# burlachenkok/flpytorch

Measured on AMD Instinct MI355X. Metric: gradient-codec encode+reduce GB/s (device-resident), [N,D] fp32; % HBM peak, higher is better.
Workload: dtype f32; 1 GPU; C3 topk:1% N=1024/GPU D=10000000; codec=topk:1%, clients_per_gpu=1024, clients_total=1024, D=10000000, K=100000, rows_alloc=contiguous, parallelism=client-shard dp1

## Files before the change

flpytorch_amd/csrc/select.hip:

```cpp
#include <stdlib.h>

#include <atomic>
#include <map>
#include <mutex>
#include <vector>

#include "chunks.hpp"
#include "randk_tree.hpp"

namespace flc {

constexpr uint32_t ALL = 0xFFFFFFFFu;
constexpr uint32_t F_OVERFLOW = 1u, F_SHORT = 2u, F_TIES = 4u, F_EXACT = 8u;
constexpr uint32_t F_RESIDENT = 16u;
constexpr uint32_t F_REPAIR = 32u;
constexpr int SMAX = 16384;
constexpr int HBINS = 2048;
constexpr uint32_t TIECAP = HBINS;
constexpr int CS_SH = 64;
constexpr int64_t CS_FEW = 16;
constexpr int CS_ST = 8;
constexpr int CS_LCAP = 2048;
constexpr int RS_U = 16;
#ifndef FLC_RS_NG
#define FLC_RS_NG 4
#endif
constexpr int RS_NG = FLC_RS_NG;
constexpr int RS_NG_MAX = 16;
static_assert(RS_NG >= 1 && RS_NG <= RS_NG_MAX, "FLC_RS_NG: 1..16 groups");
constexpr int RS_GLOB = 0, RS_GEN = 32, RS_GAVE = 64, RS_CCNT = 96, RS_CDONE = 112, RS_GRP = 128;
constexpr int RS_XGRP = RS_GRP + 32 * RS_NG_MAX;
constexpr int RS_ABV = RS_XGRP + 32 * RS_NG_MAX;
constexpr int RS_CAP = 2048;
constexpr int RS_SS = 8192;
#ifndef FLC_RS_SR
#define FLC_RS_SR 1
#endif
constexpr int RS_SR = FLC_RS_SR;
#ifndef FLC_RS_STPOL
#define FLC_RS_STPOL 2
#endif
#ifndef FLC_RS_GACQ
#define FLC_RS_GACQ 1
#endif
#ifndef FLC_RS_POLLAB
#define FLC_RS_POLLAB 1
#endif
#ifndef FLC_RS_DONE
#define FLC_RS_DONE 1
#endif
#ifndef FLC_RS_RANKFIRST
#define FLC_RS_RANKFIRST 0
#endif
#ifndef FLC_RS_PROBE_NOCOUNT
#define FLC_RS_PROBE_NOCOUNT 0
#endif
#ifndef FLC_RS_G0REL
#define FLC_RS_G0REL 1
#endif
#ifndef FLC_RS_FENCE
#define FLC_RS_FENCE 0
#endif
#ifndef FLC_RS_SPEC
#define FLC_RS_SPEC 1
#endif
constexpr int RS_HREP = RS_ABV + 32 * RS_NG_MAX;
constexpr int RS_HSPEC = RS_HREP + 3 * RS_NG * HBINS;
constexpr int RS_CLIST = RS_HSPEC + 3 * RS_NG * HBINS;
constexpr int RS_TCNT = RS_CLIST + 2 * RS_CAP;
constexpr int RS_GMAX = 1024;
constexpr int RS_CS = 4;
constexpr int RS_CNUM = RS_TCNT + 2 * RS_GMAX;
constexpr int RS_CREG = RS_CNUM + RS_GMAX;
#ifdef FLC_RS_PRINT
constexpr int RS_PROBE = RS_CREG + 2 * RS_CS * RS_GMAX;
constexpr int RS_CTL = RS_PROBE + 4096;
#else
constexpr int RS_CTL = RS_CREG + 2 * RS_CS * RS_GMAX;
#endif
#ifndef FLC_RS_SPECST
#define FLC_RS_SPECST 0
#endif
#ifndef FLC_CS_LIST
#define FLC_CS_LIST 1
#endif
#ifndef FLC_CS_TWO_MAXD
#define FLC_CS_TWO_MAXD (int64_t(64) << 20)
#endif

struct SelWs {
    uint2* tab;
    uint32_t* ent_idx;
    float* ent_val;
    uint32_t* rowcnt;
    uint32_t* flags;
    uint32_t* thr;
    uint32_t* prefix;
    uint32_t* krem;
    uint32_t* tieprefix;
    uint32_t* tiecut;
    uint32_t* hist;
    uint32_t* worklist;
    uint32_t* nwork;
    uint32_t* cursor;
    uint32_t* cstate;
    uint64_t* clist;
    uint32_t* carrive;
    uint32_t* shcnt;
    uint32_t* zm;
    float* part;
    int64_t cap;
    uint32_t tie_hi;
};

__device__ __host__ inline uint32_t tie_pref(uint32_t ix, uint32_t hi) { return hi ? ix : ~ix; }
__device__ __host__ inline uint32_t tie_all(uint32_t hi) { return hi ? 0u : 0xFFFFFFFFu; }


__device__ inline void lds_bar() {
    asm volatile("s_waitcnt lgkmcnt(0)" ::: "memory");
    __builtin_amdgcn_s_barrier();
    asm volatile("" ::: "memory");
}
template <bool RAW>
__device__ inline void blk_bar() {
    if (RAW) lds_bar();
    else __syncthreads();
}
template <bool RAW = false>
__device__ inline void hist_find_at(const uint32_t* h, uint32_t k, uint32_t& bin, uint32_t& above,
                                    uint32_t* scratch , int t, bool own) {
    uint32_t local[8];
    uint32_t s = 0;
#pragma unroll
    for (int q = 0; q < 8; ++q) { local[q] = own ? h[HBINS - 1 - (t * 8 + q)] : 0u; s += local[q]; }
    if (t == 0) { scratch[256] = 0; scratch[257] = 0; }
    const int lane = t & 63, w = t >> 6;
    uint32_t inc = s;
#pragma unroll
    for (int off = 1; off < 64; off <<= 1) {
        const uint32_t v = __shfl_up(inc, off, 64);
        inc += lane >= off ? v : 0u;
    }
    if (own && lane == 63) scratch[w] = inc;
    blk_bar<RAW>();
    uint32_t before = 0;
    if (own)
        for (int q = 0; q < w; ++q) before += scratch[q];
    uint32_t incl = own ? before + inc : 0u, excl = incl - s;
    if (own && excl < k && incl >= k) {
        uint32_t run = excl;
#pragma unroll
        for (int q = 0; q < 8; ++q) {
            if (run + local[q] >= k) {
                scratch[256] = (uint32_t)(HBINS - 1 - (t * 8 + q));
                scratch[257] = run;
                break;
            }
            run += local[q];
        }
    }
    blk_bar<RAW>();
    bin = scratch[256];
    above = scratch[257];
    blk_bar<RAW>();
}
template <int NB>
__device__ inline void hist_find_n(const uint32_t* h, uint32_t k, uint32_t& bin, uint32_t& above, bool& found,
                                   uint32_t* scratch ) {
    constexpr int PER = NB / 256;
    static_assert(NB % 256 == 0, "256 threads scan NB / 256 bins each");
    const int t = (int)threadIdx.x;
    const bool own = t < 256;
    uint32_t local[PER];
    uint32_t s = 0;
#pragma unroll
    for (int q = 0; q < PER; ++q) { local[q] = own ? h[NB - 1 - (t * PER + q)] : 0u; s += local[q]; }
    if (t == 0) { scratch[256] = 0; scratch[257] = 0; scratch[258] = 0; }
    const int lane = t & 63, w = t >> 6;
    uint32_t inc = s;
#pragma unroll
    for (int off = 1; off < 64; off <<= 1) {
        const uint32_t v = __shfl_up(inc, off, 64);
        inc += lane >= off ? v : 0u;
    }
    if (own && lane == 63) scratch[w] = inc;
    __syncthreads();
    uint32_t before = 0;
    if (own)
        for (int q = 0; q < w; ++q) before += scratch[q];
    const uint32_t incl = own ? before + inc : 0u, excl = incl - s;
    if (own && excl < k && incl >= k) {
        uint32_t run = excl;
#pragma unroll
        for (int q = 0; q < PER; ++q) {
            if (run + local[q] >= k) {
                scratch[256] = (uint32_t)(NB - 1 - (t * PER + q));
                scratch[257] = run;
                scratch[258] = 1;
                break;
            }
            run += local[q];
        }
    }
    __syncthreads();
    bin = scratch[256];
    above = scratch[257];
    found = scratch[258] != 0u;
    __syncthreads();
}
template <bool RAW = false>
__device__ inline void hist_find(const uint32_t* h, uint32_t k, uint32_t& bin, uint32_t& above,
                                 uint32_t* scratch ) {
    hist_find_at<RAW>(h, k, bin, above, scratch, (int)threadIdx.x, threadIdx.x < 256);
}
__device__ inline void hist_find2(const uint32_t* ha, uint32_t ka, uint32_t& bina, uint32_t& abovea, uint32_t* sa,
                                  const uint32_t* hb, uint32_t kb, uint32_t& binb, uint32_t& aboveb, uint32_t* sb) {
    const bool second = threadIdx.x >= 256;
    uint32_t bin, above;
    hist_find_at(second ? hb : ha, second ? kb : ka, bin, above, second ? sb : sa, (int)(threadIdx.x & 255u),
                 threadIdx.x < 512);
    bina = sa[256]; abovea = sa[257];
    binb = sb[256]; aboveb = sb[257];
    __syncthreads();
}

__device__ inline uint32_t pass_shift(int p) { return p == 0 ? 20u : (p == 1 ? 9u : 0u); }
__device__ inline uint32_t pass_bits(int p) { return p == 2 ? 9u : 11u; }
__device__ inline bool key_in_prefix(uint32_t key, int p, uint32_t prefix) {
    if (p == 0) return true;
    uint32_t sh = pass_shift(p) + pass_bits(p);
    return (key >> sh) == prefix;
}
__device__ inline uint32_t key_bin(uint32_t key, int p) {
    return (key >> pass_shift(p)) & ((1u << pass_bits(p)) - 1u);
}

template <int NT, bool DUAL>
__global__ __launch_bounds__(NT) void k_topk_sample(RowSrc rows, int64_t n, int64_t d, int64_t K, SelWs ws, int few,
                                                    int64_t r_off) {
    __shared__ uint32_t keys[SMAX];
    __shared__ uint32_t h[HBINS], h2[DUAL ? HBINS : 1];
    __shared__ uint32_t scratch[260], scratch2[DUAL ? 260 : 1];
    const int64_t row = r_off + blockIdx.x;
    if (row >= n) return;
    const float* r = rows.row(row);
    int S;
    if (d <= SMAX) {
        S = (int)d;
        for (int i = threadIdx.x; i < S; i += NT) keys[i] = mag_key(r[i]);
    } else {
        const int P = SMAX / 256;
        S = SMAX;
        constexpr int GR = NT / 256, PU = 32 / GR;
        const int e = threadIdx.x & 255, g0 = threadIdx.x >> 8;
        for (int p0 = 0; p0 < P; p0 += 32) {
            float x[PU];
#pragma unroll
            for (int u = 0; u < PU; ++u) x[u] = r[((int64_t)(p0 + u * GR + g0) * (d - 256)) / (P - 1) + e];
#pragma unroll
            for (int u = 0; u < PU; ++u) keys[(p0 + u * GR + g0) * 256 + e] = mag_key(x[u]);
        }
    }
    const int NP = S == d ? 3 : 2;
    uint32_t rank;
    if (S == d) {
        rank = (uint32_t)K;
    } else {
        double ks = (double)K * (double)S / (double)d;
        double rr = ks + 4.0 * sqrt(ks) + 8.0;
        rank = (uint32_t)min((double)S, ceil(rr));
    }
    static_assert(!DUAL || NT >= 512, "hist_find2 takes 512 threads");
    auto rank_key = [&](uint32_t r) {
        uint32_t prefix = 0, krem = r;
        for (int p = 0; p < NP; ++p) {
            for (int i = threadIdx.x; i < HBINS; i += NT) h[i] = 0;
            __syncthreads();
            for (int i = threadIdx.x; i < S; i += NT) {
                uint32_t k = keys[i];
                if (key_in_prefix(k, p, prefix)) atomicAdd(&h[key_bin(k, p)], 1u);
            }
            __syncthreads();
            uint32_t bin, above;
            hist_find(h, krem, bin, above, scratch);
            prefix = (prefix << pass_bits(p)) | bin;
            krem -= above;
            __syncthreads();
        }
        return NP == 3 ? prefix : prefix << 9;
    };
    auto rank_keys = [&](uint32_t ra, uint32_t rb, uint32_t& ka, uint32_t& kb) {
        if constexpr (!DUAL) {
            ka = rank_key(ra);
            kb = rb == ra ? ka : rank_key(rb);
            return;
        }
        uint32_t pa = 0, pb = 0, ma = ra, mb = rb;
        for (int p = 0; p < NP; ++p) {
            const bool same = pa == pb;
            for (int i = threadIdx.x; i < HBINS; i += NT) { h[i] = 0; h2[i] = 0; }
            __syncthreads();
            for (int i = threadIdx.x; i < S; i += NT) {
                const uint32_t k = keys[i];
                if (key_in_prefix(k, p, pa)) atomicAdd(&h[key_bin(k, p)], 1u);
                if (!same && key_in_prefix(k, p, pb)) atomicAdd(&h2[key_bin(k, p)], 1u);
            }
            __syncthreads();
            uint32_t ba, aa, bb, ab;
            hist_find2(h, ma, ba, aa, scratch, same ? h : h2, mb, bb, ab, scratch2);
            pa = (pa << pass_bits(p)) | ba;
            ma -= aa;
            pb = (pb << pass_bits(p)) | bb;
            mb -= ab;
        }
        ka = NP == 3 ? pa : pa << 9;
        kb = NP == 3 ? pb : pb << 9;
    };
    uint32_t tkey, kest;
    rank_keys(rank, S == d ? rank : (uint32_t)max(1.0, min((double)S, (double)K * (double)S / (double)d)), tkey, kest);
    if (threadIdx.x == 0) {
        ws.thr[row] = (rank >= (uint32_t)S && S != d) ? 0u : tkey;
        ws.prefix[row] = kest;
        ws.flags[row] = 0;
        ws.rowcnt[(row) * RCS] = 0;
        if (few) { ws.cstate[row * CS_ST + 3] = 0; ws.cstate[row * CS_ST + 5] = 0; ws.carrive[row * RCS] = 0; }
    }
    if (few && threadIdx.x < CS_SH) ws.shcnt[(row * CS_SH + threadIdx.x) * RCS] = 0;
    if (few)
        for (int i = threadIdx.x; i < HBINS; i += NT) ws.hist[row * HBINS + i] = 0;
}

#ifndef FLC_CS_NT
#define FLC_CS_NT 1
#endif
__device__ inline float4 cs_ld(const float4* p) {
#if FLC_CS_NT
    typedef float v4f __attribute__((ext_vector_type(4)));
    const v4f v = __builtin_nontemporal_load(reinterpret_cast<const v4f*>(p));
    return make_float4(v.x, v.y, v.z, v.w);
#else
    return *p;
#endif
}
template <int NT>
__device__ void cand_select_row(int64_t row, int64_t K, SelWs ws, uint32_t* h, uint32_t* scratch) {
    {
        if (ws.flags[row]) return;
        const uint32_t cnt = ws.rowcnt[(row) * RCS];
        if (cnt < (uint32_t)K) {
            if (threadIdx.x == 0) ws.flags[row] |= F_SHORT;
            return;
        }
        const uint32_t T = ws.thr[row];
        const uint32_t span = ws.prefix[row] - T;
        int s = 0;
        while (s < 21 && (((uint64_t)span * 4u) >> s) >= (uint64_t)HBINS) ++s;
        const float* vals = ws.ent_val + row * ws.cap;
        const float4* v4 = reinterpret_cast<const float4*>(vals);
        const uint32_t n4 = cnt >> 2;
        uint32_t prefix = 0, krem = (uint32_t)K, last = 0;
        bool first = true, fail = false;
        int sh = s;
        while (true) {
            const int s1 = first ? sh : max(0, sh - 11);
            const uint32_t mask = first ? 0xFFFFFFFFu : ((1u << (sh - s1)) - 1u);
            for (int i = threadIdx.x; i < HBINS; i += NT) h[i] = 0;
            __syncthreads();
            auto add = [&](float x) {
                const uint32_t dk = mag_key(x) - T;
                if (first) atomicAdd(&h[min(dk >> s1, (uint32_t)(HBINS - 1))], 1u);
                else if ((dk >> sh) == prefix) atomicAdd(&h[(dk >> s1) & mask], 1u);
            };
            uint32_t i = threadIdx.x;
            for (; i + 7 * NT < n4; i += 8 * NT) {
                float4 q[8];
#pragma unroll
                for (int u = 0; u < 8; ++u) q[u] = cs_ld(v4 + i + u * NT);
#pragma unroll
                for (int u = 0; u < 8; ++u) { add(q[u].x); add(q[u].y); add(q[u].z); add(q[u].w); }
            }
            for (; i < n4; i += NT) {
                const float4 q = v4[i];
                add(q.x); add(q.y); add(q.z); add(q.w);
            }
            for (uint32_t i = n4 * 4 + threadIdx.x; i < cnt; i += NT) add(vals[i]);
            __syncthreads();
            uint32_t bin, above;
            hist_find(h, krem, bin, above, scratch);
            last = h[bin];
            if (first && bin == HBINS - 1) { fail = true; break; }
            prefix = first ? bin : ((prefix << (sh - s1)) | bin);
            krem -= above;
            sh = s1;
            first = false;
            __syncthreads();
            if (sh == 0) break;
        }
        __syncthreads();
        const uint32_t thr = T + prefix;
        bool ties = !fail && last > krem;
        if (ties && last > TIECAP) { fail = true; ties = false; }
        if (ties) {
            uint32_t* tix = h;
            if (threadIdx.x == 0) scratch[0] = 0;
            __syncthreads();
            const uint32_t* idxs = ws.ent_idx + row * ws.cap;
            for (uint32_t i = threadIdx.x; i < n4; i += NT) {
                const float4 q = v4[i];
                const float qv[4] = {q.x, q.y, q.z, q.w};
#pragma unroll
                for (int u = 0; u < 4; ++u)
                    if (mag_key(qv[u]) == thr) tix[atomicAdd(&scratch[0], 1u)] = idxs[i * 4 + u];
            }
            for (uint32_t i = n4 * 4 + threadIdx.x; i < cnt; i += NT) {
                if (mag_key(vals[i]) == thr) tix[atomicAdd(&scratch[0], 1u)] = idxs[i];
            }
            __syncthreads();
            const uint32_t m = scratch[0];
            for (uint32_t a = threadIdx.x; a < m; a += NT) {
                const uint32_t ia = tix[a];
                uint32_t rank = 0;
                for (uint32_t b = 0; b < m; ++b) rank += tie_pref(tix[b], ws.tie_hi) > tie_pref(ia, ws.tie_hi) ? 1u : 0u;
                if (rank == krem - 1) ws.tiecut[row] = ia;
            }
        }
        if (threadIdx.x == 0) {
            if (fail) {
                ws.flags[row] |= F_SHORT;
            } else {
                ws.thr[row] = thr;
                ws.krem[row] = krem;
                if (ties) ws.flags[row] |= F_TIES;
            }
        }
        __syncthreads();
    }
}

template <int NT>
__global__ __launch_bounds__(NT) void k_cand_select(int64_t r0, int64_t rn, int64_t K, SelWs ws) {
    __shared__ uint32_t h[HBINS];
    __shared__ uint32_t scratch[260];
    for (int64_t row = r0 + blockIdx.x; row < r0 + rn; row += gridDim.x) {
        cand_select_row<NT>(row, K, ws, h, scratch);
        __syncthreads();
    }
}

constexpr int CS_NT = 256;
__global__ __launch_bounds__(CS_NT) void k_cs_pass(int64_t K, SelWs ws, int final_pass) {
    __shared__ uint32_t h[HBINS];
    __shared__ uint32_t scratch[260];
    __shared__ uint32_t last_wg;
    __shared__ uint64_t lst[FLC_CS_LIST ? CS_LCAP : 1];
    const int64_t row = blockIdx.y;
    const uint32_t B = gridDim.x, b = blockIdx.x;
    uint32_t* cs = ws.cstate + row * CS_ST;
    const uint32_t stage = cs[3];
    if (stage >= 2u) return;
    const uint32_t* shc = ws.shcnt + row * CS_SH * RCS;
    uint32_t cnt = 0;
    for (int k = 0; k < CS_SH; ++k) cnt += shc[k * RCS];
    const uint32_t mycnt = shc[b * RCS];
    const bool first = stage == 0u;
    if (first && (ws.flags[row] != 0u || cnt < (uint32_t)K)) {
        if (b == 0 && threadIdx.x == 0) {
            if (ws.flags[row] == 0u) ws.flags[row] = F_SHORT;
            cs[3] = 2u;
        }
        return;
    }
    const uint32_t T = ws.thr[row];
    uint32_t sh, prefix, krem;
    if (first) {
        const uint32_t span = ws.prefix[row] - T;
        uint32_t s0 = 0;
        while (s0 < 21 && (((uint64_t)span * 4u) >> s0) >= (uint64_t)HBINS) ++s0;
        sh = s0; prefix = 0; krem = (uint32_t)K;
    } else {
        sh = cs[0]; prefix = cs[1]; krem = cs[2];
    }
    const uint32_t s1 = first ? sh : (sh > 11u ? sh - 11u : 0u);
    const uint32_t mask = first ? 0xFFFFFFFFu : ((1u << (sh - s1)) - 1u);
    const int64_t segcap = (ws.cap / CS_SH) & ~int64_t(3);
    if (FLC_CS_LIST && !first && cs[4] <= (uint32_t)CS_LCAP) {
        if (threadIdx.x == 0) scratch[0] = 0;
        __syncthreads();
        const float* sv = ws.ent_val + row * ws.cap + b * segcap;
        const uint32_t* si = ws.ent_idx + row * ws.cap + b * segcap;
        for (uint32_t e = threadIdx.x; e < mycnt; e += CS_NT) {
            const uint32_t key = mag_key(sv[e]);
            if (((key - T) >> sh) == prefix) {
                const uint32_t slot = atomicAdd(&scratch[0], 1u);
                if (slot < (uint32_t)CS_LCAP) lst[slot] = ((uint64_t)key << 32) | (uint64_t)tie_pref(si[e], ws.tie_hi);
            }
        }
        __syncthreads();
        const uint32_t nl = min(scratch[0], (uint32_t)CS_LCAP);
        if (threadIdx.x == 0) scratch[1] = nl ? atomicAdd(&cs[5], nl) : 0u;
        __syncthreads();
        uint64_t* gl = ws.clist + row * CS_LCAP;
        const uint32_t gb = scratch[1];
        for (uint32_t i = threadIdx.x; i < nl; i += CS_NT)
            if (gb + i < (uint32_t)CS_LCAP) gl[gb + i] = lst[i];
        asm volatile("s_waitcnt vmcnt(0)" ::: "memory");
        __syncthreads();
        if (threadIdx.x == 0) {
            __builtin_amdgcn_fence(__ATOMIC_RELEASE, "agent");
            last_wg = atomicAdd(&ws.carrive[row * RCS], 1u) == B - 1u ? 1u : 0u;
        }
        __syncthreads();
        if (!last_wg) return;
        __builtin_amdgcn_fence(__ATOMIC_ACQUIRE, "agent");
        const uint32_t m = __hip_atomic_load(&cs[5], __ATOMIC_RELAXED, __HIP_MEMORY_SCOPE_AGENT);
        const bool ok = m == cs[4] && m >= krem && krem >= 1u;
        const uint32_t mm = min(m, (uint32_t)CS_LCAP);
        for (uint32_t i = threadIdx.x; i < mm; i += CS_NT)
            lst[i] = __hip_atomic_load(&gl[i], __ATOMIC_RELAXED, __HIP_MEMORY_SCOPE_AGENT);
        if (threadIdx.x == 0) { scratch[0] = 0; scratch[1] = 0; scratch[2] = 0; scratch[3] = 0; }
        __syncthreads();
        if (ok)
            for (uint32_t i = threadIdx.x; i < mm; i += CS_NT) {
                const uint64_t me = lst[i];
                uint32_t rank = 0;
                for (uint32_t j = 0; j < mm; ++j) rank += lst[j] > me ? 1u : 0u;
                if (rank == krem - 1u) { scratch[0] = (uint32_t)(me >> 32); scratch[1] = tie_pref((uint32_t)me, ws.tie_hi); }
            }
        __syncthreads();
        const uint32_t kth = scratch[0];
        if (ok)
            for (uint32_t i = threadIdx.x; i < mm; i += CS_NT) {
                const uint32_t key = (uint32_t)(lst[i] >> 32);
                if (key > kth) atomicAdd(&scratch[2], 1u);
                else if (key == kth) atomicAdd(&scratch[3], 1u);
            }
        __syncthreads();
        if (threadIdx.x == 0) {
            atomicExch(&ws.carrive[row * RCS], 0u);
            if (!ok) {
                ws.flags[row] |= F_SHORT;
            } else {
                const uint32_t gt = scratch[2], eq = scratch[3];
                ws.thr[row] = kth;
                ws.krem[row] = krem - gt;
                if (gt + eq > krem) { ws.tiecut[row] = scratch[1]; ws.flags[row] |= F_TIES; }
            }
            cs[3] = 2u;
        }
        return;
    }
    for (int i = threadIdx.x; i < HBINS; i += CS_NT) h[i] = 0;
    __syncthreads();
    auto add = [&](float x) {
        const uint32_t dk = mag_key(x) - T;
        if (first) atomicAdd(&h[min(dk >> s1, (uint32_t)(HBINS - 1))], 1u);
        else if ((dk >> sh) == prefix) atomicAdd(&h[(dk >> s1) & mask], 1u);
    };
    const float* vals = ws.ent_val + row * ws.cap + b * segcap;
    const float4* v4 = reinterpret_cast<const float4*>(vals);
    const uint32_t n4 = mycnt >> 2, q1 = n4;
    uint32_t i = threadIdx.x;
    for (; i + 3 * CS_NT < q1; i += 4 * CS_NT) {
        float4 q[4];
#pragma unroll
        for (int u = 0; u < 4; ++u) q[u] = cs_ld(v4 + i + u * CS_NT);
#pragma unroll
        for (int u = 0; u < 4; ++u) { add(q[u].x); add(q[u].y); add(q[u].z); add(q[u].w); }
    }
    for (; i < q1; i += CS_NT) {
        const float4 q = cs_ld(v4 + i);
        add(q.x); add(q.y); add(q.z); add(q.w);
    }
    for (uint32_t t = n4 * 4 + threadIdx.x; t < mycnt; t += CS_NT) add(vals[t]);
    __syncthreads();
    uint32_t* gh = ws.hist + row * HBINS;
    for (int t = threadIdx.x; t < HBINS; t += CS_NT)
        if (h[t]) atomicAdd(gh + t, h[t]);
    asm volatile("s_waitcnt vmcnt(0)" ::: "memory");
    __syncthreads();
    if (threadIdx.x == 0) {
        __builtin_amdgcn_fence(__ATOMIC_RELEASE, "agent");
        asm volatile("s_waitcnt vmcnt(0)" ::: "memory");
        last_wg = atomicAdd(&ws.carrive[row * RCS], 1u) == B - 1u ? 1u : 0u;
    }
    __syncthreads();
// ... 265 lines not shown
#pragma unroll
    for (int L = 0; L < RING - 1; ++L) {
        ring[L] = load_q(rs, lane, L);
        __builtin_amdgcn_sched_barrier(0);
    }
    const int64_t segcap = shards > 1 ? (ws.cap / shards) & ~int64_t(3) : ws.cap;
    bool pv = false;
    int64_t prow = 0, pc0 = 0, pseg = 0;
    uint64_t pcc = 0;
    uint32_t ptot = 0, pres = 0;
    int par = 0;
    auto finish = [&](int pb) {
        uint32_t base = 0;
        bool fits = ptot <= GCAP;
        if (fits && ptot) {
            base = __shfl(pres, 0, WAVE);
            fits = (int64_t)base + ptot <= segcap;
            base += (uint32_t)(pseg * segcap);
        }
        if (lane < FGS && pc0 + lane < C) {
            uint32_t off = 0, cc = 0;
#pragma unroll
            for (int u = 0; u < FGS; ++u) {
                const uint32_t cu = (uint32_t)(pcc >> (16 * u)) & 0xFFFFu;
                off += u < lane ? cu : 0u;
                cc = u == lane ? cu : cc;
            }
            ws.tab[(pc0 + lane) * n + prow] = make_uint2(base + off, fits ? cc : 0u);
        }
        if (!fits && lane == 0) atomicOr(&ws.flags[prow], F_OVERFLOW);
#if FLC_TK_COPY4
        tk_copy_out(st[pb][wv], st[pb][wv] + SROW, ws, n, prow, base, ptot, fits, lane, (int64_t)blockIdx.x * 4 + wv);
#else
        if (fits && FLC_TK_PROBE != 2) {
            const uint32_t* si = st[pb][wv];
            const float* sv = reinterpret_cast<const float*>(st[pb][wv] + SROW);
            uint32_t* oi = ws.ent_idx + prow * ws.cap + base;
            float* ov = ws.ent_val + prow * ws.cap + base;
#pragma unroll
            for (int k = 0; k < GCAP / 64; ++k) {
                const uint32_t e = (uint32_t)(k * 64 + lane);
                if (e < ptot) { oi[e] = si[e]; ov[e] = sv[e]; }
            }
        }
#endif
    };
    while (it < items) {
        const uint32_t T = max(sload(ws.thr + row), 1u);
        const int64_t nit = it + stride;
        const uint32_t sla = __builtin_amdgcn_readfirstlane((uint32_t)(size_t)(__attribute__((address_space(3))) uint32_t*)st[par][wv]);
        uint32_t cnt = 0;
        uint64_t ccp = 0;
        const int64_t cg0 = c;
        int64_t nrow = row, nc = c;
#pragma unroll
        for (int sub = 0; sub < FGS; ++sub, ++c) {
            const int64_t j0 = c * CHUNK;
            __amdgpu_buffer_rsrc_t rsn;
            if (sub + 1 < FGS) {
                rsn = chunk_rsrc(rows.row_s(row), j0 + CHUNK, d);
            } else if (nit < items) {
                item_at(nit, nrow, nc);
                rsn = chunk_rsrc(rows.row_s(nrow), nc * CHUNK, d);
            } else {
                rsn = __builtin_amdgcn_make_buffer_rsrc(const_cast<float*>(rows.row_s(row)), (short)0, 0, 0x00020000);
            }
            const uint32_t cnt0 = cnt;
            __amdgpu_buffer_rsrc_t ro;
            if constexpr (LONE != 0) ro = chunk_rsrc(zout, j0, d);
            uint32_t lb = (uint32_t)j0 + (uint32_t)lane * 4u;
            asm volatile("" : "+v"(lb));
#pragma unroll
            for (int L = 0; L < 16; ++L) {
                const int P = L + RING - 1;
                ring[P % RING] = P < 16 ? load_q(rs, lane, P) : load_q(rsn, lane, P - 16);
                const float4 x = ring[L % RING];
                if constexpr (LONE != 0) {
                    typedef unsigned int u4v __attribute__((ext_vector_type(4)));
                    const u4v z = {0u, 0u, 0u, 0u};
                    __builtin_amdgcn_raw_buffer_store_b128(z, ro, lane * 16, L * 1024, 0);
                }
                const uint32_t jl = lb + (uint32_t)(L * 256);
                const float vq[4] = {x.x, x.y, x.z, x.w};
#pragma unroll
                for (int q = 0; q < 4; ++q) {
                    if (FLC_TK_PROBE == 3) { cnt += __float_as_uint(vq[q]) == 0x7F800001u ? 1u : 0u; continue; }
                    const bool f = mag_key(vq[q]) >= T;
                    const uint64_t m = __ballot(f);
                    if (FLC_TK_PROBE != 1 && f) {
                        const uint32_t pre = __builtin_amdgcn_mbcnt_hi((uint32_t)(m >> 32), __builtin_amdgcn_mbcnt_lo((uint32_t)m, 0u));
                        uint32_t sb = sla + min(cnt, (uint32_t)GCAP) * 4u;
                        asm volatile("" : "+s"(sb));
                        asm volatile("ds_write2st64_b32 %0, %1, %2 offset1:%3" ::"v"(sb + pre * 4u),
                                     "v"(jl + q), "v"(__float_as_uint(vq[q])), "i"(SROW * 4 / 256) : "memory");
                    }
                    cnt += (uint32_t)__popcll(m);
                }
            }
            ccp |= (uint64_t)min(cnt - cnt0, 0xFFFFu) << (16 * (c - cg0));
            rs = rsn;
        }
        if (pv) finish(par ^ 1);
        uint32_t res = 0;
        const int64_t shard = shards > 1 ? (cg0 / FGS) % shards : 0;
        if (cnt && cnt <= GCAP && lane == 0)
            res = atomicAdd(shards > 1 ? &ws.shcnt[(row * shards + shard) * RCS] : &ws.rowcnt[(row) * RCS], cnt);
        pv = true; prow = row; pc0 = cg0; pcc = ccp; ptot = cnt; pres = res; pseg = shard;
        __builtin_amdgcn_fence(__ATOMIC_SEQ_CST, "wavefront");
        par ^= 1;
        it = nit;
        row = nrow;
        c = nc;
    }
    __builtin_amdgcn_fence(__ATOMIC_SEQ_CST, "wavefront");
    finish(par ^ 1);
}

#ifndef FLC_TK_WG
#define FLC_TK_WG 1
#endif
#ifndef FLC_TK_WG_NL
#define FLC_TK_WG_NL 4
#endif
#ifndef FLC_TK_WG_RING
#define FLC_TK_WG_RING FLC_TK_RING
#endif
#ifndef FLC_TK_WG_STPOL
#define FLC_TK_WG_STPOL 17
#endif
#ifndef FLC_TK_WG_WPE
#define FLC_TK_WG_WPE 4
#endif
__device__ inline uint32_t lds_addr(const void* p) {
    return (uint32_t)(size_t)(const __attribute__((address_space(3))) void*)p;
}
__device__ inline uint32_t lds_peek(uint32_t addr) {
    uint32_t v;
    asm volatile("ds_read_b32 %0, %1\n\ts_waitcnt lgkmcnt(0)" : "=&v"(v) : "v"(addr) : "memory");
    return __builtin_amdgcn_readfirstlane(v);
}
template <int RING, int NL>
__global__ __launch_bounds__((NL + 1) * 64) __attribute__((amdgpu_waves_per_eu(FLC_TK_WG_WPE))) void k_topk_filter_fast_wg(RowSrc rows, int64_t n, int64_t r0, int64_t rn, int64_t rb, int64_t d,
                                                                        SelWs ws) {
    static_assert(16 % RING == 0, "ring must divide the 16 loads of a chunk");
    constexpr int FGS = 4;
    constexpr int SROW = GCAP + 64;
    __shared__ __attribute__((aligned(16))) uint32_t st[2][NL][2 * SROW];
    __shared__ __attribute__((aligned(16))) uint32_t hs[2][NL][4];
    __shared__ uint32_t fr[2];
    const int lane = threadIdx.x & 63;
    const int wv = __builtin_amdgcn_readfirstlane(threadIdx.x >> 6);
    if (threadIdx.x < 2 * NL * 4) (&hs[0][0][0])[threadIdx.x] = 0;
    if (threadIdx.x < 2) fr[threadIdx.x] = 0;
    __syncthreads();
    const int64_t C = nchunks(d);
    const int64_t G = (C + FGS * NL - 1) / (FGS * NL);
    const int64_t items = rn * G;
    const int64_t stride = gridDim.x;
    int64_t it = blockIdx.x;
    if (it >= items) return;
    auto item_at = [&](int64_t t, int64_t& r, int64_t& cc) {
        const int64_t blk = t / (rb * G), rem = t - blk * rb * G;
        const int64_t bn = min(rb, rn - blk * rb);
        const int64_t g = rem / bn;
        r = r0 + blk * rb + (rem - g * bn);
        cc = g * (FGS * NL);
    };
    if (wv == NL) {
        for (uint32_t k = 0; it < items; it += stride, ++k) {
            const int b = k & 1;
            int64_t row, c0;
            item_at(it, row, c0);
            const uint32_t fa = lds_addr(&hs[b][min(lane, NL - 1)][3]);
            for (;;) {
                uint32_t f;
                asm volatile("ds_read_b32 %0, %1\n\ts_waitcnt lgkmcnt(0)" : "=&v"(f) : "v"(fa) : "memory");
                if (__ballot(f != k + 1) == 0) break;
                __builtin_amdgcn_s_sleep(4);
            }
            uint32_t pre[NL], tot[NL], sum = 0;
            uint64_t cc[NL];
            bool allfit = true;
#pragma unroll
            for (int w = 0; w < NL; ++w) {
                const uint4 h = *reinterpret_cast<const uint4*>(hs[b][w]);
                cc[w] = (uint64_t)h.x | ((uint64_t)h.y << 32);
                tot[w] = h.z;
                pre[w] = sum;
                sum += tot[w] <= GCAP ? tot[w] : 0u;
                allfit = allfit && tot[w] <= GCAP;
            }
            uint32_t base = 0;
            bool fits = true;
            if (sum) {
                uint32_t res = 0;
                if (lane == 0) res = atomicAdd(&ws.rowcnt[row * RCS], sum);
                base = __shfl(res, 0, WAVE);
                fits = (int64_t)base + sum <= ws.cap;
            }
            if (lane < FGS * NL && c0 + lane < C) {
                uint32_t off = 0, cu = 0;
                bool gf = false;
#pragma unroll
                for (int w = 0; w < NL; ++w)
                    if ((lane >> 2) == w) {
                        off = pre[w];
                        gf = tot[w] <= GCAP;
#pragma unroll
                        for (int u = 0; u < FGS; ++u) {
                            const uint32_t x = (uint32_t)(cc[w] >> (16 * u)) & 0xFFFFu;
                            off += u < (lane & 3) ? x : 0u;
                            cu = u == (lane & 3) ? x : cu;
                        }
                    }
                ws.tab[(c0 + lane) * n + row] = make_uint2(base + off, fits && gf ? cu : 0u);
            }
            if (!(fits && allfit) && lane == 0) atomicOr(&ws.flags[row], F_OVERFLOW);
#pragma unroll
            for (int w = 0; w < NL; ++w)
                tk_copy_out<FLC_TK_WG_STPOL>(st[b][w], st[b][w] + SROW, ws, n, row, base + pre[w], tot[w], fits && tot[w] <= GCAP, lane,
                            (int64_t)blockIdx.x * NL + w);
            asm volatile("s_waitcnt lgkmcnt(0)\n\tds_write_b32 %0, %1" ::"v"(lds_addr(&fr[b])), "v"(k + 1) : "memory");
        }
        return;
    }
    float4 ring[RING];
    int64_t row, c;
    item_at(it, row, c);
    c += wv * FGS;
    auto rs = chunk_rsrc(rows.row_s(row), c * CHUNK, d);
#pragma unroll
    for (int L = 0; L < RING - 1; ++L) {
        ring[L] = load_q(rs, lane, L);
        __builtin_amdgcn_sched_barrier(0);
    }
    for (uint32_t k = 0; it < items; ++k) {
        const int b = k & 1;
        if (k >= 2) {
            const uint32_t fa = lds_addr(&fr[b]);
            while (lds_peek(fa) != k - 1) __builtin_amdgcn_s_sleep(2);
        }
        const uint32_t T = max(sload(ws.thr + row), 1u);
        const int64_t nit = it + stride;
        const uint32_t sla = __builtin_amdgcn_readfirstlane(lds_addr(st[b][wv]));
        uint32_t cnt = 0;
        uint64_t ccp = 0;
        const int64_t cg0 = c;
        int64_t nrow = row, nc = c;
#pragma unroll
        for (int sub = 0; sub < FGS; ++sub, ++c) {
            const int64_t j0 = c * CHUNK;
            __amdgpu_buffer_rsrc_t rsn;
            if (sub + 1 < FGS) {
                rsn = chunk_rsrc(rows.row_s(row), j0 + CHUNK, d);
            } else if (nit < items) {
                item_at(nit, nrow, nc);
                nc += wv * FGS;
                rsn = chunk_rsrc(rows.row_s(nrow), nc * CHUNK, d);
            } else {
                rsn = __builtin_amdgcn_make_buffer_rsrc(const_cast<float*>(rows.row_s(row)), (short)0, 0, 0x00020000);
            }
            const uint32_t cnt0 = cnt;
            uint32_t lb = (uint32_t)j0 + (uint32_t)lane * 4u;
            asm volatile("" : "+v"(lb));
#pragma unroll
            for (int L = 0; L < 16; ++L) {
                const int P = L + RING - 1;
                ring[P % RING] = P < 16 ? load_q(rs, lane, P) : load_q(rsn, lane, P - 16);
                const float4 x = ring[L % RING];
                const uint32_t jl = lb + (uint32_t)(L * 256);
                const float vq[4] = {x.x, x.y, x.z, x.w};
#pragma unroll
                for (int q = 0; q < 4; ++q) {
                    const bool f = mag_key(vq[q]) >= T;
                    const uint64_t m = __ballot(f);
                    if (f) {
                        const uint32_t pre = __builtin_amdgcn_mbcnt_hi((uint32_t)(m >> 32), __builtin_amdgcn_mbcnt_lo((uint32_t)m, 0u));
                        uint32_t sb = sla + min(cnt, (uint32_t)GCAP) * 4u;
                        asm volatile("" : "+s"(sb));
                        asm volatile("ds_write2st64_b32 %0, %1, %2 offset1:%3" ::"v"(sb + pre * 4u),
                                     "v"(jl + q), "v"(__float_as_uint(vq[q])), "i"(SROW * 4 / 256) : "memory");
                    }
                    cnt += (uint32_t)__popcll(m);
                }
            }
            ccp |= (uint64_t)min(cnt - cnt0, 0xFFFFu) << (16 * (c - cg0));
            rs = rsn;
        }
        if (lane == 0)
            asm volatile("ds_write_b64 %0, %1\n\tds_write_b32 %0, %2 offset:8\n\tds_write_b32 %0, %3 offset:12"
                         ::"v"(lds_addr(hs[b][wv])), "v"(ccp), "v"(cnt), "v"(k + 1) : "memory");
        it = nit;
        row = nrow;
        c = nc;
    }
}

template <bool FULLROW>
__global__ __launch_bounds__(256) void k_radix_hist(RowSrc rows, int64_t n, int64_t d, int p, SelWs ws) {
    __shared__ uint32_t h[HBINS];
    constexpr int64_t BLK = 65536;
    const int64_t nrows = FULLROW ? (int64_t)(*ws.nwork) : n;
    const int64_t maxlen = FULLROW ? d : ws.cap;
    const int64_t bpr = (maxlen + BLK - 1) / BLK;
    const int64_t items = nrows * bpr;
    for (int64_t it = blockIdx.x; it < items; it += gridDim.x) {
        const int64_t li = it / bpr;
        const int64_t row = FULLROW ? (int64_t)ws.worklist[li] : li;
        if (!FULLROW && ws.flags[row]) continue;
        const int64_t len = FULLROW ? d : (int64_t)ws.rowcnt[(row) * RCS];
        const int64_t b0 = (it % bpr) * BLK;
        if (b0 >= len) continue;
        const int64_t b1 = min(len, b0 + BLK);
        for (int i = threadIdx.x; i < HBINS; i += 256) h[i] = 0;
        __syncthreads();
        const uint32_t prefix = ws.prefix[row];
        const float* src = FULLROW ? rows.row(row) : (ws.ent_val + row * ws.cap);
        for (int64_t j = b0 + threadIdx.x; j < b1; j += 256) {
            const uint32_t k = mag_key(src[j]);
            if (key_in_prefix(k, p, prefix)) atomicAdd(&h[key_bin(k, p)], 1u);
        }
        __syncthreads();
        uint32_t* gh = ws.hist + row * HBINS;
        for (int i = threadIdx.x; i < HBINS; i += 256)
            if (h[i]) atomicAdd(&gh[i], h[i]);
        __syncthreads();
    }
}

template <bool FULLROW>
__global__ __launch_bounds__(256) void k_radix_select(int64_t n, int p, int64_t K, SelWs ws) {
    __shared__ uint32_t scratch[260];
    const int64_t nrows = FULLROW ? (int64_t)(*ws.nwork) : n;
    for (int64_t li = blockIdx.x; li < nrows; li += gridDim.x) {
        const int64_t row = FULLROW ? (int64_t)ws.worklist[li] : li;
        if (!FULLROW && ws.flags[row]) continue;
        uint32_t* gh = ws.hist + row * HBINS;
        if (!FULLROW && p == 0 && ws.rowcnt[(row) * RCS] < (uint32_t)K) {
            for (int i = threadIdx.x; i < HBINS; i += 256) gh[i] = 0;
            if (threadIdx.x == 0) ws.flags[row] |= F_SHORT;
            continue;
        }
        const uint32_t k = (p == 0) ? (uint32_t)K : ws.krem[row];
        uint32_t bin, above;
        hist_find(gh, k, bin, above, scratch);
        const uint32_t ties_here = gh[bin];
        __syncthreads();
        for (int i = threadIdx.x; i < HBINS; i += 256) gh[i] = 0;
        if (threadIdx.x == 0) {
            const uint32_t pre = (p == 0) ? 0u : ws.prefix[row];
            ws.prefix[row] = (pre << pass_bits(p)) | bin;
            ws.krem[row] = k - above;
            if (p == 2) {
                ws.thr[row] = ws.prefix[row];
                if (FULLROW) ws.tiecut[row] = ties_here;
                if (ties_here > k - above) ws.flags[row] |= (FULLROW ? F_TIES | F_EXACT : F_TIES);
                else if (FULLROW) ws.flags[row] |= F_EXACT;
            }
        }
        __syncthreads();
    }
}

__global__ void k_build_worklist(int64_t n, int64_t K, int64_t d, SelWs ws, int force_all) {
    __shared__ uint32_t cnt;
    if (threadIdx.x == 0) cnt = 0;
    __syncthreads();
    for (int64_t row = threadIdx.x; row < n; row += blockDim.x) {
        uint32_t f = ws.flags[row];
        if (force_all || (f & (F_OVERFLOW | F_SHORT))) {
// ... 2574 lines not shown
```

Baseline: 5914 GB/s.

## Build coarse candidate histogram during filter to enable one-pass top-k threshold select

The filter kernel's writer wave now bins each surviving candidate into a 64-bin coarse histogram, kept per row in global memory. The candidate-select step then reads this histogram to find the coarse bin holding the K-th element. It gathers only that bin's low key bits into LDS and refines the threshold there, replacing repeated full re-reads of the candidate buffer with one read. This adds LDS and global atomics to the filter's copy-out path and falls back to the multi-pass loop when the bin overflows or the counts disagree.

```diff
diff --git a/flpytorch_amd/csrc/select.hip b/flpytorch_amd/csrc/select.hip
--- a/flpytorch_amd/csrc/select.hip
+++ b/flpytorch_amd/csrc/select.hip
@@ -21,6 +21,7 @@
 constexpr int64_t CS_FEW = 16;
 constexpr int CS_ST = 8;
 constexpr int CS_LCAP = 2048;
+constexpr int CS_CB = 64;
 constexpr int RS_U = 16;
 #ifndef FLC_RS_NG
 #define FLC_RS_NG 4
@@ -326,6 +327,7 @@
         ws.rowcnt[(row) * RCS] = 0;
         if (few) { ws.cstate[row * CS_ST + 3] = 0; ws.cstate[row * CS_ST + 5] = 0; ws.carrive[row * RCS] = 0; }
     }
+    if (!few && threadIdx.x < CS_CB) ws.hist[row * HBINS + threadIdx.x] = 0;
     if (few && threadIdx.x < CS_SH) ws.shcnt[(row * CS_SH + threadIdx.x) * RCS] = 0;
     if (few)
         for (int i = threadIdx.x; i < HBINS; i += NT) ws.hist[row * HBINS + i] = 0;
@@ -343,6 +345,127 @@
     return *p;
 #endif
 }
+__device__ inline int cs_first_shift(uint32_t span) {
+    int s = 0;
+    while (s < 21 && (((uint64_t)span * 4u) >> s) >= (uint64_t)HBINS) ++s;
+    return s;
+}
+
+#ifndef FLC_CS_ONEPASS
+#define FLC_CS_ONEPASS 1
+#endif
+#ifndef FLC_CS_PROBE
+#define FLC_CS_PROBE 0
+#endif
+constexpr uint32_t F_ONEPASS = 64u;
+constexpr int CS_CW = 4;
+constexpr int CS_OLCAP = 1536;
+constexpr int CS_ONB = HBINS - CS_OLCAP;
+static_assert(CS_ONB == 512 && CS_CB == WAVE, "one-pass select: 512 histogram bins, one coarse bin a lane");
+__device__ inline uint32_t cs_onepass_cap(int cs) { return cs <= 16 ? 2u * CS_OLCAP : (uint32_t)CS_OLCAP; }
+
+template <int NT>
+__device__ bool cand_select_onepass(int64_t row, int64_t K, const SelWs& ws, uint32_t* h, uint32_t* scratch, uint32_t cnt,
+                                    uint32_t T, int s, uint32_t& prefix, uint32_t& krem, uint32_t& last) {
+    const int cs = s + CS_CW;
+    if (threadIdx.x < CS_CB) {
+        const int lane = (int)threadIdx.x;
+        const uint32_t c = ws.hist[row * HBINS + lane];
+        uint32_t inc = c;
+#pragma unroll
+        for (int off = 1; off < 64; off <<= 1) {
+            const uint32_t v = __shfl_down(inc, off, 64);
+            inc += lane + off < 64 ? v : 0u;
+        }
+        const uint32_t total = __shfl(inc, 0, 64);
+        if (lane == 0) { scratch[0] = 0; scratch[4] = 0; }
+        if (total == cnt && inc >= (uint32_t)K && inc - c < (uint32_t)K && lane != CS_CB - 1 && c <= cs_onepass_cap(cs)) {
+            scratch[0] = 1; scratch[1] = (uint32_t)lane; scratch[2] = inc - c; scratch[3] = c;
+        }
+    }
+    __syncthreads();
+    if (!scratch[0]) { __syncthreads(); return false; }
+    const uint32_t cb = scratch[1], above = scratch[2], expect = scratch[3];
+    const float* vals = ws.ent_val + row * ws.cap;
+    const float4* v4 = reinterpret_cast<const float4*>(vals);
+    const uint32_t n4 = cnt >> 2;
+    const bool half = cs <= 16;
+    const uint32_t lowmask = (1u << cs) - 1u, cap = cs_onepass_cap(cs);
+    uint16_t* h16 = reinterpret_cast<uint16_t*>(h);
+    auto put = [&](uint32_t pos, uint32_t dk) {
+        if (pos < cap) {
+            if (half) h16[pos] = (uint16_t)(dk & lowmask);
+            else h[pos] = dk & lowmask;
+        }
+    };
+    auto take = [&](float x) {
+        const uint32_t dk = mag_key(x) - T;
+        if ((dk >> cs) == cb) put(atomicAdd(&scratch[4], 1u), dk);
+    };
+    auto round8 = [&](uint32_t i, auto part) {
+        float4 q[8];
+        uint32_t valid = 0xFFFFFFFFu;
+#pragma unroll
+        for (int u = 0; u < 8; ++u) {
+            if (!decltype(part)::value || i + u * NT < n4) q[u] = cs_ld(v4 + i + u * NT);
+            else { q[u] = make_float4(0.f, 0.f, 0.f, 0.f); valid &= ~(0xFu << (4 * u)); }
+        }
+        __builtin_amdgcn_sched_barrier(0);
+        uint32_t hits = 0;
+#pragma unroll
+        for (int u = 7; u >= 0; --u) {
+            const float qv[4] = {q[u].x, q[u].y, q[u].z, q[u].w};
+#pragma unroll
+            for (int c = 3; c >= 0; --c) hits = (hits << 1) | (((mag_key(qv[c]) - T) >> cs) == cb ? 1u : 0u);
+        }
+        hits &= valid;
+        if (hits) {
+            uint32_t pos = atomicAdd(&scratch[4], (uint32_t)__popc(hits));
+#pragma unroll
+            for (int u = 0; u < 8; ++u) {
+                const float qv[4] = {q[u].x, q[u].y, q[u].z, q[u].w};
+#pragma unroll
+                for (int c = 0; c < 4; ++c)
+                    if ((hits >> (u * 4 + c)) & 1u) put(pos++, mag_key(qv[c]) - T);
+            }
+        }
+    };
+    uint32_t i = threadIdx.x;
+    for (; i + 7 * NT < n4; i += 8 * NT) round8(i, std::false_type{});
+    if (i < n4) round8(i, std::true_type{});
+    for (uint32_t j = n4 * 4 + threadIdx.x; j < cnt; j += NT) take(vals[j]);
+    __syncthreads();
+    const uint32_t m = scratch[4];
+    __syncthreads();
+    if (m != expect) return false;
+    uint32_t* hb = h + CS_OLCAP;
+    uint32_t pfx = 0, kr = (uint32_t)K - above;
+    int sh = cs;
+    while (sh > 0) {
+        const int s1 = max(0, sh - 9);
+        const uint32_t mask = (1u << (sh - s1)) - 1u;
+        for (int b = threadIdx.x; b < CS_ONB; b += NT) hb[b] = 0;
+        __syncthreads();
+        for (uint32_t a = threadIdx.x; a < m; a += NT) {
+            const uint32_t lo = half ? (uint32_t)h16[a] : h[a];
+            if ((lo >> sh) == pfx) atomicAdd(&hb[(lo >> s1) & mask], 1u);
+        }
+        __syncthreads();
+        uint32_t bin, ab;
+        bool found;
+        hist_find_n<CS_ONB>(hb, kr, bin, ab, found, scratch);
+        last = hb[bin];
+        pfx = (pfx << (sh - s1)) | bin;
+        kr -= ab;
+        sh = s1;
+        __syncthreads();
+    }
+    pfx |= cb << cs;
+    prefix = pfx;
+    krem = kr;
+    return true;
+}
+
 template <int NT>
 __device__ void cand_select_row(int64_t row, int64_t K, SelWs ws, uint32_t* h, uint32_t* scratch) {
     {
@@ -353,16 +476,18 @@
             return;
         }
         const uint32_t T = ws.thr[row];
-        const uint32_t span = ws.prefix[row] - T;
-        int s = 0;
-        while (s < 21 && (((uint64_t)span * 4u) >> s) >= (uint64_t)HBINS) ++s;
+        const int s = cs_first_shift(ws.prefix[row] - T);
         const float* vals = ws.ent_val + row * ws.cap;
         const float4* v4 = reinterpret_cast<const float4*>(vals);
         const uint32_t n4 = cnt >> 2;
         uint32_t prefix = 0, krem = (uint32_t)K, last = 0;
         bool first = true, fail = false;
         int sh = s;
-        while (true) {
+        bool one = false;
+#if FLC_CS_ONEPASS && !FLC_CS_PROBE
+        one = cand_select_onepass<NT>(row, K, ws, h, scratch, cnt, T, s, prefix, krem, last);
+#endif
+        while (!one) {
             const int s1 = first ? sh : max(0, sh - 11);
             const uint32_t mask = first ? 0xFFFFFFFFu : ((1u << (sh - s1)) - 1u);
             for (int i = threadIdx.x; i < HBINS; i += NT) h[i] = 0;
@@ -372,7 +497,7 @@
                 if (first) atomicAdd(&h[min(dk >> s1, (uint32_t)(HBINS - 1))], 1u);
                 else if ((dk >> sh) == prefix) atomicAdd(&h[(dk >> s1) & mask], 1u);
             };
-            uint32_t i = threadIdx.x;
+            uint32_t i = FLC_CS_PROBE == 1 && first ? n4 : threadIdx.x;
             for (; i + 7 * NT < n4; i += 8 * NT) {
                 float4 q[8];
 #pragma unroll
@@ -388,6 +513,7 @@
             __syncthreads();
             uint32_t bin, above;
             hist_find(h, krem, bin, above, scratch);
+            if (FLC_CS_PROBE == 1 && first) { bin = 3 * HBINS / 16; above = 0; }
             last = h[bin];
             if (first && bin == HBINS - 1) { fail = true; break; }
             prefix = first ? bin : ((prefix << (sh - s1)) | bin);
@@ -431,7 +557,7 @@
             } else {
                 ws.thr[row] = thr;
                 ws.krem[row] = krem;
-                if (ties) ws.flags[row] |= F_TIES;
+                if (ties || one) ws.flags[row] |= (ties ? F_TIES : 0u) | (one ? F_ONEPASS : 0u);
             }
         }
         __syncthreads();
@@ -1003,6 +1129,10 @@
     const int wv = __builtin_amdgcn_readfirstlane(threadIdx.x >> 6);
     if (threadIdx.x < 2 * NL * 4) (&hs[0][0][0])[threadIdx.x] = 0;
     if (threadIdx.x < 2) fr[threadIdx.x] = 0;
+#if FLC_CS_ONEPASS
+    __shared__ uint32_t ch[CS_CB];
+    if (threadIdx.x < CS_CB) ch[threadIdx.x] = 0;
+#endif
     __syncthreads();
     const int64_t C = nchunks(d);
     const int64_t G = (C + FGS * NL - 1) / (FGS * NL);
@@ -1067,6 +1197,29 @@
                 ws.tab[(c0 + lane) * n + row] = make_uint2(base + off, fits && gf ? cu : 0u);
             }
             if (!(fits && allfit) && lane == 0) atomicOr(&ws.flags[row], F_OVERFLOW);
+#if FLC_CS_ONEPASS
+            {
+                const uint32_t Tr = ws.thr[row];
+                const uint32_t csh = (uint32_t)(cs_first_shift(ws.prefix[row] - Tr) + CS_CW);
+                uint32_t c63 = 0;
+#pragma unroll
+                for (int w = 0; w < NL; ++w) {
+                    const uint32_t tw = (fits && tot[w] <= GCAP) ? __builtin_amdgcn_readfirstlane(tot[w]) : 0u;
+                    const uint32_t* sv = st[b][w] + SROW;
+                    for (uint32_t e0 = 0; e0 < tw; e0 += 64) {
+                        const uint32_t e = e0 + (uint32_t)lane;
+                        const bool in = e < tw;
+                        const uint32_t cbn = min(((sv[in ? e : 0u] & 0x7FFFFFFFu) - Tr) >> csh, (uint32_t)(CS_CB - 1));
+                        c63 += (uint32_t)__popcll(__ballot(in && cbn == CS_CB - 1));
+                        if (in && cbn != CS_CB - 1) atomicAdd(&ch[cbn], 1u);
+                    }
+                }
+                __builtin_amdgcn_fence(__ATOMIC_SEQ_CST, "wavefront");
+                const uint32_t cl = ch[lane] + (lane == CS_CB - 1 ? c63 : 0u);
+                ch[lane] = 0;
+                if (cl) atomicAdd(&ws.hist[row * HBINS + lane], cl);
+            }
+#endif
 #pragma unroll
             for (int w = 0; w < NL; ++w)
                 tk_copy_out<FLC_TK_WG_STPOL>(st[b][w], st[b][w] + SROW, ws, n, row, base + pre[w], tot[w], fits && tot[w] <= GCAP, lane,
```

Result: no change. 5966 GB/s (median of 6 runs) (+0.9%).
